# RobotLocomotion/pytorch-dense-correspondence

Hardware: NVIDIA H100
Metric: image-pairs/s (640x480, D=3) fwd+loss+bwd (higher is better)
Workload: dtype f32 (bf16x3 split on the wgmma tensor cores, fp32 accumulate)

## Files before the change

include/ddn_b200.h:

```cpp
#ifndef DDN_B200_H_
#define DDN_B200_H_

#include <stddef.h>
#include <stdint.h>

#ifdef __cplusplus
extern "C" {
#endif

#define DDN_ABI_VERSION 3

enum {
  DDN_OK = 0,
  DDN_EINVAL = -1,
  DDN_EWORKSPACE = -2,
  DDN_EUNSUPPORTED = -3
};

enum {
  DDN_PRECISION_FP32_SIMT = 0,
  DDN_PRECISION_BF16X3 = 1,
  DDN_PRECISION_BF16 = 2
};

// ... 151 lines not shown
                               float* five_host );

int ddn_conv2d_forward(const float* x_nhwc, const float* w_oihw, float* y_nhwc,
                       int N, int H, int W, int Cin, int Cout, int k, int stride, int pad, int dil,
                       int precision, void* workspace, size_t workspace_bytes, void* stream);
size_t ddn_conv2d_workspace_bytes(int N, int H, int W, int Cin, int Cout, int k, int stride, int pad, int dil, int precision);
int ddn_conv2d_backward(const float* x_nhwc, const float* w_oihw, const float* dy_nhwc,
                        float* dx_nhwc, float* dw_oihw,
                        int N, int H, int W, int Cin, int Cout, int k, int stride, int pad, int dil,
                        int precision, void* workspace, size_t workspace_bytes, void* stream);

int ddn_batchnorm_forward(const float* x, const float* gamma, const float* beta, const float* residual,
                          float* y, float* save_mean, float* save_invstd,
                          float* running_mean, float* running_var,
                          int64_t M, int C, int relu, int training, float momentum, float eps,
                          void* workspace, size_t workspace_bytes, void* stream);
int ddn_batchnorm_backward(const float* dy, const float* x, const float* y, const float* gamma,
                           const float* save_mean, const float* save_invstd,
                           float* dx, float* dgamma, float* dbeta, float* d_residual,
                           int64_t M, int C, int relu, void* workspace, size_t workspace_bytes, void* stream);
size_t ddn_batchnorm_workspace_bytes(int64_t M, int C);

size_t ddn_conv2d_fused_workspace_bytes(int N, int H, int W, int Cin, int Cout, int k, int stride, int pad, int dil, int precision);
int ddn_conv2d_bn_stats_forward(const float* x_nhwc, const float* w_oihw, float* raw_nhwc, float* mean, float* invstd,
                                float* running_mean, float* running_var,
                                int N, int H, int W, int Cin, int Cout, int k, int stride, int pad, int dil,
                                int bn_groups, float momentum, float eps, int precision,
                                void* workspace, size_t workspace_bytes, void* stream);
int ddn_conv2d_folded_forward(const float* x_nhwc, const float* w_oihw, const float* gamma, const float* beta,
                              const float* running_mean, const float* running_var, const float* addend_nhwc,
                              float* y_nhwc, void* y_hi_bf16, void* y_lo_bf16,
                              int N, int H, int W, int Cin, int Cout, int k, int stride, int pad, int dil, int relu, float eps,
                              int precision, void* workspace, size_t workspace_bytes, void* stream);
int ddn_conv2d_backward_data_bn_stats(const float* w_oihw, const float* dy_nhwc, const float* addend_nhwc,
                                      const float* raw_nhwc, const float* mean, const float* invstd, const float* gamma,
                                      const float* beta, const void* y_hi_bf16,
                                      float* dx_nhwc, float* dgamma, float* dbeta, float* sums,
                                      int N, int H, int W, int Cin, int Cout, int k, int stride, int pad, int dil,
                                      int bn_groups, int precision, void* workspace, size_t workspace_bytes, void* stream);

int ddn_stem_pool_forward(const float* raw, const float* mean, const float* invstd, const float* gamma, const float* beta,
                          float* y, void* y_hi_bf16, void* y_lo_bf16, void* argmax_u8, int N, int Hc, int Wc, int G, void* stream);
size_t ddn_stem_workspace_bytes(int N, int H, int W, int precision);
int ddn_stem_backward(const float* x_nchw, const float* raw, const float* mean, const float* invstd, const float* gamma,
                      const float* beta, const void* argmax_u8, const float* dy_pool, float* g_out, float* dx_bn,
                      void* dx_hi_bf16, void* dx_lo_bf16, float* dgamma, float* dbeta, float* dw_conv1,
// ... 188 lines not shown
```

pytorch-dense-correspondence_b200/_native.py:

```python
import ctypes
import os

import torch

_HERE = os.path.dirname(os.path.abspath(__file__))
LIB_PATH = os.path.join(_HERE, "libddn_b200.so")

PRECISION_FP32_SIMT, PRECISION_BF16X3, PRECISION_BF16 = 0, 1, 2
MODE_INFER, MODE_TRAIN, MODE_EVAL_SAVE = 0, 1, 2
ARCH_RESNET34_8S, ARCH_RESNET50_8S = 0, 1
GRAD_BUCKET_FN = ctypes.CFUNCTYPE(None, ctypes.c_void_p, ctypes.c_int, ctypes.c_int64, ctypes.c_int64)
TERM_MATCH, TERM_HINGE, TERM_HINGE_INV = 0, 1, 2
TERM_PIXEL_WEIGHT = 1
NET_UNIT_DESCRIPTORS = 1
LOWRES_UNIT = 1
MAX_TERMS = 8

c_f32p = ctypes.POINTER(ctypes.c_float)
vp, i32, i64, f32, sz = ctypes.c_void_p, ctypes.c_int, ctypes.c_int64, ctypes.c_float, ctypes.c_size_t


class TensorEntry(ctypes.Structure):
    _fields_ = [("name", ctypes.c_char * 64), ("ndim", ctypes.c_int32), ("shape", ctypes.c_int32 * 4),
                ("offset", ctypes.c_int64), ("numel", ctypes.c_int64)]
# ... 103 lines not shown
    "ddn_net_param_table": (i32, [i32, i32, ctypes.POINTER(TensorEntry), i32]),
    "ddn_net_buffer_table": (i32, [i32, ctypes.POINTER(TensorEntry), i32]),
    "ddn_net_param_count": (i64, [i32, i32]),
    "ddn_net_buffer_count": (i64, [i32]),
    "ddn_net_workspace_bytes": (sz, [i32] * 7),
    "ddn_net_weight_cache_bytes": (sz, [i32, i32]),
    "ddn_net_forward": (i32, [i32, vp, vp, vp, vp, vp, sz, i32, i32, i32, i32, i32, i32, f32, f32, i32, vp, vp]),
    "ddn_net_backward": (i32, [i32, vp, vp, vp, vp, vp, sz, i32, i32, i32, i32, i32, i32, f32, i32, GRAD_BUCKET_FN, vp, vp]),
    "ddn_net_grad_buckets": (i32, [i32, i32, ctypes.POINTER(i64), i32]),
    "ddn_net_workspace_bytes_v2": (sz, [i32] * 8),
    "ddn_net_forward_v2": (i32, [i32, vp, vp, vp, vp, vp, sz, i32, i32, i32, i32, i32, i32, f32, f32, i32, vp, i32, vp]),
    "ddn_net_backward_v2": (i32, [i32, vp, vp, vp, vp, vp, sz, i32, i32, i32, i32, i32, i32, f32, i32, i32, GRAD_BUCKET_FN, vp, vp]),
    "ddn_contrastive_terms_forward": (i32, [vp, vp, i64, i64, i64, i32, i64, i32, i32, ctypes.POINTER(LossTerm), i32, vp, vp, vp]),
    "ddn_contrastive_terms_backward": (i32, [vp, vp, i64, i64, i64, i32, i64, i32, i32, ctypes.POINTER(LossTerm), i32,
                                             vp, vp, vp, vp, vp]),
    "ddn_within_scene_compose": (i32, [vp, vp, i32, i32, ctypes.POINTER(WithinSceneCfg), vp, vp, vp]),
    "ddn_pair_type_compose": (i32, [vp, vp, i32, i32, ctypes.POINTER(PairTypeComposeCfg), vp, vp, vp, vp]),
    "ddn_within_scene_loss_host": (i32, [vp, vp, i32, i32, i32, i32, vp, vp, i64, vp, vp, i64, vp, vp, i64,
                                         f32, f32, f32, f32, i32, vp]),
    "ddn_conv2d_workspace_bytes": (sz, [i32] * 10),
    "ddn_conv2d_forward": (i32, [vp, vp, vp] + [i32] * 10 + [vp, sz, vp]),
    "ddn_conv2d_backward": (i32, [vp, vp, vp, vp, vp] + [i32] * 10 + [vp, sz, vp]),
    "ddn_conv2d_fused_workspace_bytes": (sz, [i32] * 10),
    "ddn_conv2d_bn_stats_forward": (i32, [vp] * 7 + [i32] * 10 + [f32, f32, i32, vp, sz, vp]),
    "ddn_conv2d_folded_forward": (i32, [vp] * 10 + [i32] * 10 + [f32, i32, vp, sz, vp]),
    "ddn_conv2d_backward_data_bn_stats": (i32, [vp] * 13 + [i32] * 11 + [vp, sz, vp]),
    "ddn_stem_pool_forward": (i32, [vp] * 9 + [i32] * 4 + [vp]),
    "ddn_stem_workspace_bytes": (sz, [i32] * 4),
    "ddn_stem_backward": (i32, [vp] * 15 + [i32] * 6 + [vp, sz, vp]),
    "ddn_batchnorm_workspace_bytes": (sz, [i64, i32]),
    "ddn_batchnorm_forward": (i32, [vp] * 9 + [i64, i32, i32, i32, f32, f32, vp, sz, vp]),
    "ddn_batchnorm_backward": (i32, [vp] * 10 + [i64, i32, i32, vp, sz, vp]),
    "ddn_upsample_bilinear_forward": (i32, [vp, vp, i32, i32, i32, i32, i32, vp]),
    "ddn_upsample_bilinear_backward": (i32, [vp, vp, i32, i32, i32, i32, i32, vp]),
    "ddn_upsample_bilinear_unit_forward": (i32, [vp, vp, i32, i32, i32, i32, i32, i32, vp]),
    "ddn_upsample_bilinear_unit_backward": (i32, [vp, vp, vp, vp, i32, i32, i32, i32, i32, i32, vp]),
    "ddn_fc_workspace_bytes": (sz, [i32, i32]),
    "ddn_fc_forward": (i32, [vp] * 7 + [i64, i32, i32, i32, vp]),
    "ddn_fc_backward": (i32, [vp] * 8 + [i64, i32, i32, i32, vp, sz, vp]),
    "ddn_scale_inplace": (i32, [vp, i64, f32, vp]),
    "ddn_sample_non_matches_scratch_bytes": (sz, [i32, i32]),
    "ddn_sample_non_matches": (i32, [vp, i32, i32, vp, vp, i64, vp, i64, vp, vp, vp, sz, vp]),
    "ddn_find_pixel_correspondences_scratch_bytes": (sz, [i64]),
    "ddn_find_pixel_correspondences": (i32, [vp, vp, i32, i32, vp, i64, vp, vp, vp, vp, vp, vp, vp, vp, vp, sz, vp]),
    "ddn_within_scene_batch_scratch_bytes": (sz, [ctypes.POINTER(WsBatchCfg)]),
    "ddn_within_scene_batch": (i32, [ctypes.POINTER(WsBatchCfg)] + [vp] * 9 + [ctypes.POINTER(WsBatchRand),
# ... 116 lines not shown
```

pytorch-dense-correspondence_b200/csrc/conv_tc.cu:

```cuda
#include <cuda.h>
#include <algorithm>
#include <cstring>
#include <functional>
#include <mutex>
#include <unordered_map>

#include "conv.cuh"
#include "conv_tc.cuh"

namespace ddn {

constexpr int TC_BLOCK_K = 64;
constexpr int TC_CONSUMERS = 256;
constexpr int TC_THREADS = TC_CONSUMERS + 32;
constexpr int TC_PRODUCER_WARP = TC_CONSUMERS / 32;
constexpr int TC_WIDE_THREADS = TC_CONSUMERS + 128;
constexpr int TC_A_BYTES = 128 * TC_BLOCK_K * 2;

__device__ __forceinline__ uint32_t smem_u32(const void* p) { return (uint32_t)__cvta_generic_to_shared(p); }

__device__ __forceinline__ void mbar_init(uint32_t bar, uint32_t count) {
  asm volatile("mbarrier.init.shared::cta.b64 [%0], %1;" ::"r"(bar), "r"(count));
}
__device__ __forceinline__ void mbar_expect_tx(uint32_t bar, uint32_t bytes) {
// ... 261 lines not shown

__device__ __forceinline__ void named_barrier(int id, int threads) { asm volatile("bar.sync %0, %1;" ::"r"(id), "r"(threads) : "memory"); }

__device__ __forceinline__ void conv_epilogue_finalize(const TcEpilogueParams& p, int C, int* s_last, int bar) {
  if (p.fin.a.acc) {
    if (bn_last_cta(p.fin.a.ticket, gridDim.x, threadIdx.x == 0, s_last, [bar] { named_barrier(bar, TC_CONSUMERS); }))
      for (int c = threadIdx.x; c < C; c += TC_CONSUMERS) bn_fwd_finalize_channel(p.fin, c);
  } else if (p.bst.fin.a.acc) {
    if (bn_last_cta(p.bst.fin.a.ticket, gridDim.x, threadIdx.x == 0, s_last, [bar] { named_barrier(bar, TC_CONSUMERS); }))
      for (int c = threadIdx.x; c < C; c += TC_CONSUMERS) bn_bwd_finalize_channel(p.bst.fin, c);
  }
}

struct TcConvParams {
  TcEpilogueParams epi;
  int N, H, W, Cin, Cout;
  int taps_w;
  int dil;
  int stride;
  int tiles_h, tiles_w;
  int n_sub;
  int n_co;
  int full_items, tail_split, total_items;
};

constexpr int TC_SUB_H = 4, TC_SUB_W = 16;
constexpr int TC_SUB_BYTES = 64 * 128;

struct TcItem { int sp, co0, width; };
__device__ __forceinline__ TcItem tc_item(const TcConvParams& p, int idx, int block_n) {
  int tile = idx, piece = 0, width = block_n;
  if (idx >= p.full_items) {
    const int j = idx - p.full_items;
    tile = p.full_items + j / p.tail_split;
    piece = j - (j / p.tail_split) * p.tail_split;
    width = block_n / p.tail_split;
  }
  TcItem it;
  it.sp = tile / p.n_co;
  it.co0 = (tile - it.sp * p.n_co) * block_n + piece * width;
  it.width = width;
  return it;
}
struct TcSub { int n, h0, w0; bool valid; };
__device__ __forceinline__ TcSub tc_sub(const TcConvParams& p, int st) {
  TcSub s;
  s.valid = st < p.n_sub;
  const int tw = st % p.tiles_w; const int t = st / p.tiles_w;
  const int th = t % p.tiles_h;
  s.n = s.valid ? t / p.tiles_h : p.N;
// ... 12 lines not shown
  constexpr int K_STEP = TRANS ? 16 * 128 : 32;
  for (int kb = 0; kb < num_kb; ++kb, ++g) {
    const int s = g % STAGES;
    mbar_wait(smem_u32(&full_bar[s]), (g / STAGES) & 1);
    wgmma_fence();
    const uint32_t stg = smem_u32(smem + (size_t)s * STAGE_BYTES);
    const uint64_t a_hi = gmma_desc(stg + wg * TC_SUB_BYTES, LBO, 1024), a_lo = gmma_desc(stg + A_BYTES + wg * TC_SUB_BYTES, LBO, 1024);
    const uint64_t b_hi = gmma_desc(stg + NSPLIT * A_BYTES, LBO, 1024), b_lo = gmma_desc(stg + 2 * A_BYTES + B_BYTES, LBO, 1024);
#pragma unroll
    for (int k = 0; k < TC_BLOCK_K / 16; ++k) {
      const uint64_t adv = (uint64_t)((k * K_STEP) >> 4);
      mma_k16_x<W, TRANS, NPROD>(acc, accx, a_hi + adv, a_lo + adv, b_hi + adv, b_lo + adv, (kb | k) != 0);
    }
    wgmma_commit();
    wgmma_wait<1>();
    if (kb > 0 && lane == 0) mbar_arrive(smem_u32(&empty_bar[(g - 1) % STAGES]));
  }
  wgmma_wait<0>();
  fence_acc(acc);
  if (NPROD == 3) { fence_acc(accx); add_cross(acc, accx); }
  if (lane == 0) mbar_arrive(smem_u32(&empty_bar[(g - 1) % STAGES]));
}

template <int BLOCK_N, int NPROD>
__global__ void __launch_bounds__(TC_WIDE_THREADS, 1)
conv_tc_kernel(const __grid_constant__ CUtensorMap tm_a_hi, const __grid_constant__ CUtensorMap tm_a_lo,
               const __grid_constant__ CUtensorMap tm_b_hi, const __grid_constant__ CUtensorMap tm_b_lo,
               const __grid_constant__ CUtensorMap tm_bt_hi, const __grid_constant__ CUtensorMap tm_bt_lo,
               const TcConvParams p) {
  constexpr int NSPLIT = NPROD == 3 ? 2 : 1;
  constexpr int A_BYTES = 128 * TC_BLOCK_K * 2;
  constexpr int B_BYTES = BLOCK_N * TC_BLOCK_K * 2;
  constexpr int STAGE_BYTES = NSPLIT * (A_BYTES + B_BYTES);
  constexpr int STAGES = (192 * 1024) / STAGE_BYTES >= 8 ? 8 : (192 * 1024) / STAGE_BYTES;
  static_assert(STAGES >= 2, "pipeline needs at least two stages");

  extern __shared__ __align__(1024) uint8_t smem_raw[];
  uint8_t* smem = reinterpret_cast<uint8_t*>((reinterpret_cast<uintptr_t>(smem_raw) + 1023) & ~uintptr_t(1023));
  __shared__ __align__(8) uint64_t full_bar[STAGES];
  __shared__ __align__(8) uint64_t empty_bar[STAGES];
  __shared__ int s_last;
  __shared__ __align__(16) float s_stage[TC_CONSUMERS / 32][EPI_WARP_FLOATS];
  __shared__ __align__(16) float s_part[2][2][4][BLOCK_N];

  pdl_trigger();
  const int warp = __shfl_sync(0xffffffffu, threadIdx.x >> 5, 0), lane = threadIdx.x & 31;
  const int cin_chunks = p.Cin / TC_BLOCK_K;
  const int num_kb = p.taps_w * p.taps_w * cin_chunks;
  const int half = p.taps_w >> 1;

  if (threadIdx.x == 0) {
    for (int s = 0; s < STAGES; ++s) { mbar_init(smem_u32(&full_bar[s]), 1); mbar_init(smem_u32(&empty_bar[s]), TC_CONSUMERS / 32); }
    fence_barrier_init();
    tma_prefetch_desc(&tm_a_hi); tma_prefetch_desc(&tm_b_hi); tma_prefetch_desc(&tm_bt_hi);
    if (NSPLIT == 2) { tma_prefetch_desc(&tm_a_lo); tma_prefetch_desc(&tm_b_lo); tma_prefetch_desc(&tm_bt_lo); }
  }
  __syncthreads();
  pdl_wait();

  if (warp >= TC_PRODUCER_WARP) {
    setmaxnreg_dec<40>();
    if (warp == TC_PRODUCER_WARP && lane == 0) {
      uint32_t g = 0;
      for (int idx = blockIdx.x; idx < p.total_items; idx += gridDim.x) {
        const TcItem it = tc_item(p, idx, BLOCK_N);
        const bool tail = it.width != BLOCK_N;
        const uint32_t stage_tx = (uint32_t)(NSPLIT * (A_BYTES + it.width * TC_BLOCK_K * 2));
        const CUtensorMap* mb_hi = tail ? &tm_bt_hi : &tm_b_hi;
        const CUtensorMap* mb_lo = tail ? &tm_bt_lo : &tm_b_lo;
        const TcSub s0 = tc_sub(p, it.sp * 2), s1 = tc_sub(p, it.sp * 2 + 1);
        for (int kb = 0; kb < num_kb; ++kb, ++g) {
          const int s = g % STAGES;
          mbar_wait(smem_u32(&empty_bar[s]), ((g / STAGES) & 1) ^ 1);
          const int tap = kb / cin_chunks, cc = kb - tap * cin_chunks;
          const int r = tap / p.taps_w, sx = tap - r * p.taps_w;
          const int dh = (r - half) * p.dil, dw = (sx - half) * p.dil;
          uint8_t* stg = smem + (size_t)s * STAGE_BYTES;
          const uint32_t bar = smem_u32(&full_bar[s]);
          mbar_expect_tx(bar, stage_tx);
          tma_load_4d(smem_u32(stg), &tm_a_hi, bar, cc * TC_BLOCK_K, s0.w0 * p.stride + dw, s0.h0 * p.stride + dh, s0.n);
          tma_load_4d(smem_u32(stg + TC_SUB_BYTES), &tm_a_hi, bar, cc * TC_BLOCK_K, s1.w0 * p.stride + dw, s1.h0 * p.stride + dh, s1.n);
          tma_load_2d(smem_u32(stg + NSPLIT * A_BYTES), mb_hi, bar, kb * TC_BLOCK_K, it.co0);
          if (NSPLIT == 2) {
            tma_load_4d(smem_u32(stg + A_BYTES), &tm_a_lo, bar, cc * TC_BLOCK_K, s0.w0 * p.stride + dw, s0.h0 * p.stride + dh, s0.n);
            tma_load_4d(smem_u32(stg + A_BYTES + TC_SUB_BYTES), &tm_a_lo, bar, cc * TC_BLOCK_K, s1.w0 * p.stride + dw, s1.h0 * p.stride + dh, s1.n);
            tma_load_2d(smem_u32(stg + 2 * A_BYTES + B_BYTES), mb_lo, bar, kb * TC_BLOCK_K, it.co0);
          }
        }
      }
    }
  } else {
    setmaxnreg_inc<232>();
    const int wg = warp >> 2, w = warp & 3, e = threadIdx.x & 127;
    const int ga = lane >> 3, gb = lane & 7;
    const bool stats = p.epi.fin.a.acc != nullptr;
    const bool bstats = p.epi.bst.fin.a.acc != nullptr;
    double* const sum_acc = bstats ? p.epi.bst.fin.a.acc : p.epi.fin.a.acc;
    float* const st = s_stage[warp];
    float acc[BLOCK_N / 2], accx[BLOCK_N / 2];
    uint32_t g = 0;
    for (int idx = blockIdx.x; idx < p.total_items; idx += gridDim.x) {
      const TcItem it = tc_item(p, idx, BLOCK_N);
      if (it.width == BLOCK_N)
        conv_tc_mainloop<BLOCK_N, BLOCK_N, NPROD, STAGES>(acc, accx, num_kb, g, full_bar, empty_bar, smem, wg, lane);
      else if (BLOCK_N > 64 && it.width == 64)
        conv_tc_mainloop<64, BLOCK_N, NPROD, STAGES>(acc_cols<64>(acc), acc_cols<64>(accx), num_kb, g, full_bar, empty_bar, smem, wg, lane);
      else
        conv_tc_mainloop<32, BLOCK_N, NPROD, STAGES>(acc_cols<32>(acc), acc_cols<32>(accx), num_kb, g, full_bar, empty_bar, smem, wg, lane);

      const TcSub sb = tc_sub(p, it.sp * 2 + wg);
      const int h = sb.h0 + w, w4 = sb.w0 + EPI_ROWS * ga;
      const int n_ok = (sb.valid && h < p.H) ? min(EPI_ROWS, p.W - w4) : 0;
      const size_t pix = ((size_t)(n_ok > 0 ? sb.n : 0) * p.H + (n_ok > 0 ? h : 0)) * p.W + (n_ok > 0 ? w4 : 0);
      const size_t cbase = pix * p.Cout + it.co0 + gb * 4;
      const int grp = sb.valid ? sb.n / p.epi.imgs_per_group : 0;
#pragma unroll
      for (int c = 0; c < BLOCK_N / 32; ++c) {
        if (c < (it.width >> 5)) {
          float4 v[EPI_ROWS];
          stage_chunk(acc, c, st, lane, v);
          float4 s1 = make_float4(0.f, 0.f, 0.f, 0.f), s2 = s1;
          conv_epilogue_rows(p.epi, v, cbase + c * 32, (size_t)p.Cout, n_ok, it.co0 + c * 32 + gb * 4, p.Cout, grp, s1, s2);
          if (stats || bstats) {
            colsum_lane_groups(s1, s2);
            if (ga == 0) {
              *reinterpret_cast<float4*>(&s_part[wg][0][w][c * 32 + gb * 4]) = s1;
              *reinterpret_cast<float4*>(&s_part[wg][1][w][c * 32 + gb * 4]) = s2;
            }
          }
        }
      }
      if (stats || bstats) {
        named_barrier(1 + wg, 128);
        if (sb.valid)
          for (int col = e; col < it.width; col += 128) {
#pragma unroll
            for (int k = 0; k < 2; ++k) {
              const float sum = s_part[wg][k][0][col] + s_part[wg][k][1][col] + s_part[wg][k][2][col] + s_part[wg][k][3][col];
              red_add_f64(sum_acc + (size_t)(grp * 2 + k) * p.Cout + it.co0 + col, (double)sum);
            }
          }
        named_barrier(1 + wg, 128);
      }
    }
    conv_epilogue_finalize(p.epi, p.Cout, &s_last, 3);
// ... 836 lines not shown
  DDN_CHECK_ARG(n % 4 == 0, "split: element count must be a multiple of 4");
  int64_t n4 = n / 4;
  int blocks = (int)std::min<int64_t>(ceil_div(n4, 256), (int64_t)num_sms() * 8);
  DDN_LAUNCH(split_bf16_kernel, blocks, 256, 0, st, x, hi, lo, n4, precision == DDN_PRECISION_BF16X3 ? 1 : 0);
  return 0;
}

int tc_upsample_zero_split(const float* dy, __nv_bfloat16* hi, __nv_bfloat16* lo, int N, int Ho, int Wo, int C, int precision,
                           cudaStream_t st) {
  int64_t total = (int64_t)N * Ho * Wo * (C / 4);
  int blocks = (int)std::min<int64_t>(ceil_div(total, 256), (int64_t)num_sms() * 8);
  DDN_LAUNCH(upsample_zero_split_kernel, blocks, 256, 0, st, dy, hi, lo, N, Ho, Wo, C, precision == DDN_PRECISION_BF16X3 ? 1 : 0);
  return 0;
}

int tc_stem_patches(const float* x_nchw, __nv_bfloat16* hi, __nv_bfloat16* lo, int N, int H, int W, int precision, cudaStream_t st) {
  const int H1 = (H - 1) / 2 + 1, W1 = (W - 1) / 2 + 1;
  DDN_CHECK_ARG(N <= 65535 && H1 <= 65535, "stem: batch / height too large for the launch grid");
  dim3 grid((unsigned)ceil_div(W1, STEM_TW), (unsigned)H1, (unsigned)N);
  DDN_LAUNCH(stem_patch_split_kernel, grid, 256, 0, st, x_nchw, hi, lo, N, H, W, H1, W1, precision == DDN_PRECISION_BF16X3 ? 1 : 0);
  return 0;
}

template <int BLOCK_N, int NPROD>
static int launch_conv_tc(const CUtensorMap& a_hi, const CUtensorMap& a_lo, const CUtensorMap& b_hi, const CUtensorMap& b_lo,
                          const CUtensorMap& bt_hi, const CUtensorMap& bt_lo, const TcConvParams& p, int workers, cudaStream_t st) {
  constexpr int NSPLIT = NPROD == 3 ? 2 : 1;
  constexpr int STAGE_BYTES = NSPLIT * (128 * TC_BLOCK_K * 2 + BLOCK_N * TC_BLOCK_K * 2);
  constexpr int STAGES = (192 * 1024) / STAGE_BYTES >= 8 ? 8 : (192 * 1024) / STAGE_BYTES;
  const size_t smem = (size_t)STAGES * STAGE_BYTES + 1024;
  static bool configured = false;
  if (!configured) {
    DDN_CUDA(cudaFuncSetAttribute(conv_tc_kernel<BLOCK_N, NPROD>, cudaFuncAttributeMaxDynamicSharedMemorySize, (int)smem));
    configured = true;
  }
  DDN_LAUNCH((conv_tc_kernel<BLOCK_N, NPROD>), workers, TC_WIDE_THREADS, smem, st, a_hi, a_lo, b_hi, b_lo, bt_hi, bt_lo, p);
  return 0;
}

template <int NPROD>
static int launch_conv64_halo(const CUtensorMap& a_hi, const CUtensorMap& a_lo, const CUtensorMap& b_hi, const CUtensorMap& b_lo,
                              const TcHaloParams& p, cudaStream_t st) {
  constexpr int NSPLIT = NPROD == 3 ? 2 : 1;
  const size_t smem = (size_t)NSPLIT * HALO_B_PLANE + (size_t)halo_slots(NPROD) * HALO_SLOT + 1024;
  static bool configured = false;
  if (!configured) {
    DDN_CUDA(cudaFuncSetAttribute(conv64_halo_kernel<NPROD>, cudaFuncAttributeMaxDynamicSharedMemorySize, (int)smem));
    configured = true;
  }
  const int grid = std::min(p.n_tiles, tc_worker_sms());
  DDN_LAUNCH((conv64_halo_kernel<NPROD>), grid, TC_THREADS, smem, st, a_hi, a_lo, b_hi, b_lo, p);
  return 0;
}

static int tc_epilogue_request(TcEpilogueParams* e, float* out, const float* addend, const BnFwdFinal* stats, const TcBwdStats* bst,
                               const TcFoldedEpilogue* ep, int N, int gout, int dgrad, int want_lo) {
  memset(e, 0, sizeof(*e));
  e->out = out; e->addend = addend; e->imgs_per_group = N;
  if (stats) {
// ... 54 lines not shown
    DDN_TRY(make_weight_map(&mb_lo, want_lo ? b_lo : b_hi, 64, 9 * 64, 64));
    ProfScope ps(dgrad ? PROF_CONV_DGRAD_TC : PROF_CONV_FWD_TC, fl, st);
    return want_lo ? launch_conv64_halo<3>(ma_hi, ma_lo, mb_hi, mb_lo, hp, st) : launch_conv64_halo<1>(ma_hi, ma_lo, mb_hi, mb_lo, hp, st);
  }
  const int block_n = gout % 128 == 0 ? 128 : 64;
  TcConvParams p;
  memset(&p, 0, sizeof(p));
  p.epi = epi; p.N = N; p.H = Ho; p.W = Wo; p.Cin = gin; p.Cout = gout; p.taps_w = k; p.dil = dil;
  p.stride = stride;
  p.tiles_h = (int)ceil_div(Ho, TC_SUB_H); p.tiles_w = (int)ceil_div(Wo, TC_SUB_W);
  p.n_sub = N * p.tiles_h * p.tiles_w;
  p.n_co = gout / block_n;
  const int tiles = (int)ceil_div(p.n_sub, 2) * p.n_co;
  const int workers_max = tc_worker_sms();
  const int rem = tiles % workers_max;
  int split = 1;
  if (rem)
    while (split * 2 <= 8 && block_n / (split * 2) >= 32 && rem * split * 2 <= workers_max) split *= 2;
  p.full_items = tiles - rem; p.tail_split = split; p.total_items = p.full_items + rem * split;
  if (split == 1) { p.full_items = tiles; p.total_items = tiles; }
  const int workers = std::min(p.total_items, workers_max);
  const int b_rows = block_n;
  const int bt_rows = b_rows / split;
  CUtensorMap ma_hi, ma_lo, mb_hi, mb_lo, mt_hi, mt_lo;
  DDN_TRY(make_act_map(&ma_hi, in.hi, N, H, W, gin, stride));
  DDN_TRY(make_act_map(&ma_lo, want_lo ? in.lo : in.hi, N, H, W, gin, stride));
  DDN_TRY(make_weight_map(&mb_hi, b_hi, gout, k * k * gin, b_rows));
  DDN_TRY(make_weight_map(&mb_lo, want_lo ? b_lo : b_hi, gout, k * k * gin, b_rows));
  DDN_TRY(make_weight_map(&mt_hi, b_hi, gout, k * k * gin, bt_rows));
  DDN_TRY(make_weight_map(&mt_lo, want_lo ? b_lo : b_hi, gout, k * k * gin, bt_rows));
  ProfScope ps(dgrad ? PROF_CONV_DGRAD_TC : PROF_CONV_FWD_TC, fl, st);
#define CONV_TC(BN)                                                                                                           \
  (want_lo ? launch_conv_tc<BN, 3>(ma_hi, ma_lo, mb_hi, mb_lo, mt_hi, mt_lo, p, workers, st)                                   \
           : launch_conv_tc<BN, 1>(ma_hi, ma_lo, mb_hi, mb_lo, mt_hi, mt_lo, p, workers, st))
  if (block_n == 128) return CONV_TC(128);
  return CONV_TC(64);
#undef CONV_TC
}

int tc_dgrad_strided(const float* dy_f32, TcPlanes up, const float* w_oihw, const TcPlanes* w_packed, float* dx, const float* addend,
                     int N, int H, int W, int Cin, int Cout, int k, int precision, void* wws, size_t wws_bytes, cudaStream_t st,
                     const TcBwdStats* bst) {
  DDN_TRY(tc_upsample_zero_split(dy_f32, const_cast<__nv_bfloat16*>(up.hi), const_cast<__nv_bfloat16*>(up.lo), N, H / 2, W / 2, Cout,
                                 precision, st));
  return tc_conv_planes(up, w_oihw, w_packed, dx, addend, nullptr, N, H, W, Cin, Cout, k, 1, 1, 1, precision, wws, wws_bytes, st, nullptr, bst);
}

int tc_stem_pack_weights(const float* w_conv1, __nv_bfloat16* hi, __nv_bfloat16* lo, int precision, cudaStream_t st) {
  DDN_LAUNCH(stem_pack_weights_kernel, (64 * 192 + 255) / 256, 256, 0, st, w_conv1, hi, lo, precision == DDN_PRECISION_BF16X3 ? 1 : 0);
  return 0;
}
int tc_stem_forward(TcPlanes patches, const float* w_conv1, const TcPlanes* w_packed, float* raw, const BnFwdFinal* stats, int N, int H1,
                    int W1, int precision, void* wws, size_t wws_bytes, cudaStream_t st) {
  TcPlanes wpk;
  if (w_packed) wpk = *w_packed;
  else {
    char* base = reinterpret_cast<char*>(align_up(reinterpret_cast<uintptr_t>(wws), 1024));
    DDN_CHECK_ARG((size_t)(base - (char*)wws) + 2 * 64 * 192 * 2 + 1024 <= wws_bytes, "weight staging too small");
    __nv_bfloat16* ph = (__nv_bfloat16*)base; __nv_bfloat16* pl = (__nv_bfloat16*)(base + align_up((size_t)64 * 192 * 2, 1024));
// ... 71 lines not shown
```

pytorch-dense-correspondence_b200/csrc/conv_tc.cuh:

```cuda
#pragma once
#include "common.cuh"
#include "bn_stats.cuh"

namespace ddn {

struct TcPlanes { const __nv_bfloat16* hi; const __nv_bfloat16* lo; };

struct TcFoldedEpilogue { const float* scale; const float* shift; int relu; __nv_bfloat16* out_hi; __nv_bfloat16* out_lo; };

struct TcBwdStats {
  const float* raw; const __nv_bfloat16* y_hi;
  const float* mean; const float* invstd;
  const float* gamma; const float* beta;
  int relu;
  BnBwdFinal fin;
};

bool tc_conv_supported(int Cin, int Cout, int k, int stride, int pad, int dil, int H, int W);
size_t tc_weight_ws_bytes();
size_t tc_max_weight_elems();
size_t tc_workspace_bytes(size_t max_act_elems);
int tc_split(const float* x, __nv_bfloat16* hi, __nv_bfloat16* lo, int64_t n, int precision, cudaStream_t st);

int tc_conv_planes(TcPlanes in, const float* w_oihw, const TcPlanes* w_packed, float* out, const float* addend, const BnFwdFinal* stats,
                   int N, int H, int W, int Cin, int Cout, int k, int stride, int dil, int dgrad, int precision,
                   void* wws, size_t wws_bytes, cudaStream_t st, const TcFoldedEpilogue* ep = nullptr, const TcBwdStats* bst = nullptr);
int tc_dgrad_strided(const float* dy_f32, TcPlanes up, const float* w_oihw, const TcPlanes* w_packed, float* dx, const float* addend,
                     int N, int H, int W, int Cin, int Cout, int k, int precision, void* wws, size_t wws_bytes, cudaStream_t st,
                     const TcBwdStats* bst = nullptr);
int tc_wgrad_planes(TcPlanes x, TcPlanes dy, float* dw, int N, int H, int W, int Cin, int Cout, int k, int stride, int dil,
                    int precision, double* dwp, cudaStream_t st);
struct TcUnpackEntry { int64_t src_off, dst_off; int Cout, Cin, taps, kind; };
constexpr int TC_UNPACK_MAX = 40;
struct TcUnpackTable { TcUnpackEntry e[TC_UNPACK_MAX]; int n; };
int tc_unpack_wgrads(const TcUnpackEntry* entries, int n, const double* dwp_base, float* grads_base, cudaStream_t st);
struct TcPackEntry { int64_t w_off, dst_off; int Cout, Cin, k, dgrad, kind; };
constexpr int TC_PACK_MAX = 80;
struct TcPackTable { TcPackEntry e[TC_PACK_MAX]; int n; };
int tc_pack_all(const float* params, int64_t n_params, char* cache, const TcPackEntry* entries, int n, unsigned long long* fp_new,
                unsigned long long* fp_old, int force, int precision, cudaStream_t st);
int tc_stem_patches(const float* x_nchw, __nv_bfloat16* hi, __nv_bfloat16* lo, int N, int H, int W, int precision, cudaStream_t st);
int tc_stem_pack_weights(const float* w_conv1, __nv_bfloat16* hi, __nv_bfloat16* lo, int precision, cudaStream_t st);
// ... 13 lines not shown
```

pytorch-dense-correspondence_b200/csrc/engine.cu:

```cuda
#include <algorithm>
#include <cstring>
#include <deque>
#include <mutex>
#include <string>
#include <vector>

#include "conv.cuh"
#include "conv_tc.cuh"

namespace ddn {

std::atomic<long long> g_launches{0};
static thread_local char g_err[512] = "";

void set_error(const char* fmt, ...) {
  va_list ap;
  va_start(ap, fmt);
  vsnprintf(g_err, sizeof(g_err), fmt, ap);
  va_end(ap);
}

static std::atomic<int> g_reserved_sms{-1};
static std::atomic<int> g_window_reserved{0};
static int overlap_window_sms() {
// ... 963 lines not shown
  BnBwdArgs a;
  memset(&a, 0, sizeof(a));
  a.dy = dy; a.x = x; a.mean = save_mean; a.invstd = save_invstd; a.gamma = gamma; a.y = y;
  a.dx = dx; a.g_out = d_residual; a.dgamma = dgamma; a.dbeta = dbeta;
  a.acc = bn_accum_at(workspace, C); a.sums = reinterpret_cast<float*>((char*)workspace + bn_accum_bytes(C));
  a.M = M; a.C = C; a.relu = relu; a.training = 1; a.G = 1;
  return launch_bn_backward(a, st);
}

static bool is_stem_shape(int Cin, int Cout, int k, int stride, int pad, int dil) {
  return Cin == 3 && Cout == 64 && k == 7 && stride == 2 && pad == 3 && dil == 1;
}
static size_t fused_head_bytes(int C) { return bn_accum_bytes(C) + align_up(sizeof(float) * 2 * (size_t)C, 256); }

extern "C" size_t ddn_conv2d_fused_workspace_bytes(int N, int H, int W, int Cin, int Cout, int k, int stride, int pad, int dil,
                                                   int precision) {
  if (N < 1 || H < 1 || W < 1 || Cin < 1 || Cout < 1 || precision == DDN_PRECISION_FP32_SIMT) return 0;
  const int C = Cin > Cout ? Cin : Cout;
  size_t act = (size_t)N * H * W * C;
  if (is_stem_shape(Cin, Cout, k, stride, pad, dil)) act = (size_t)N * conv_out(H, 7, 2, 3, 1) * conv_out(W, 7, 2, 3, 1) * 192;
  return fused_head_bytes(C) + tc_workspace_bytes(act) + 1024;
}

static int check_fused(int N, int H, int W, int Cin, int Cout, int k, int stride, int pad, int dil, int G, int precision,
                       size_t ws_bytes, bool allow_stem) {
  DDN_CHECK_ARG(precision >= DDN_PRECISION_FP32_SIMT && precision <= DDN_PRECISION_BF16, "unknown precision %d", precision);
  if (precision == DDN_PRECISION_FP32_SIMT) {
    set_error("the fused conv epilogues exist on the tensor-core path only (precision %d)", precision);
    return DDN_EUNSUPPORTED;
  }
  DDN_CHECK_ARG(N >= 1 && H >= 8 && W >= 8, "bad sizes N=%d H=%d W=%d", N, H, W);
  DDN_CHECK_ARG(G >= 1 && G <= BN_MAX_GROUPS && N % G == 0, "bn_groups must be 1 or %d and divide N (got %d for N=%d)", BN_MAX_GROUPS, G, N);
  const bool stem = is_stem_shape(Cin, Cout, k, stride, pad, dil);
  if (stem) {
    if (!allow_stem) { set_error("the stem patch GEMM has no fused variant here"); return DDN_EUNSUPPORTED; }
  } else if (!tc_conv_supported(Cin, Cout, k, stride, pad, dil, H, W)) {
    set_error("shape not supported by the tensor-core path (Cin=%d Cout=%d k=%d stride=%d pad=%d dil=%d H=%d W=%d)", Cin, Cout, k, stride,
              pad, dil, H, W);
    return DDN_EUNSUPPORTED;
  }
  DDN_CHECK_ARG(ws_bytes >= ddn_conv2d_fused_workspace_bytes(N, H, W, Cin, Cout, k, stride, pad, dil, precision), "workspace too small");
  return 0;
}

extern "C" int ddn_conv2d_bn_stats_forward(const float* x, const float* w, float* raw, float* mean, float* invstd, float* running_mean,
                                           float* running_var, int N, int H, int W, int Cin, int Cout, int k, int stride, int pad,
// ... 158 lines not shown
```

Baseline: 139.6.

## Load one haloed activation row box per kernel row for 3x3 dgrad convs

For stride-1 3x3 data-gradient convolutions, the producer now loads one wider activation box per kernel row (with dilation halo) and reuses it for all three horizontal taps by shifting the wgmma descriptor. Activation and weight tiles get separate mbarrier rings, with weights still streamed per tap. This cuts activation TMA traffic about threefold for these layers. In exchange, the shared-memory split and epilogue indexing change (column-major sub-tile rows), which adds complexity and leaves fewer weight stages.

```diff
diff --git a/include/ddn_b200.h b/include/ddn_b200.h
--- a/include/ddn_b200.h
+++ b/include/ddn_b200.h
@@ -197,6 +197,7 @@
 size_t ddn_batchnorm_workspace_bytes(int64_t M, int C);
 
 size_t ddn_conv2d_fused_workspace_bytes(int N, int H, int W, int Cin, int Cout, int k, int stride, int pad, int dil, int precision);
+int ddn_conv_tc_load_bytes(int k, int stride, int dil, int dgrad, int width, int precision, int64_t* out);
 int ddn_conv2d_bn_stats_forward(const float* x_nhwc, const float* w_oihw, float* raw_nhwc, float* mean, float* invstd,
                                 float* running_mean, float* running_var,
                                 int N, int H, int W, int Cin, int Cout, int k, int stride, int pad, int dil,
diff --git a/pytorch-dense-correspondence_b200/_native.py b/pytorch-dense-correspondence_b200/_native.py
--- a/pytorch-dense-correspondence_b200/_native.py
+++ b/pytorch-dense-correspondence_b200/_native.py
@@ -149,6 +149,7 @@
     "ddn_conv2d_forward": (i32, [vp, vp, vp] + [i32] * 10 + [vp, sz, vp]),
     "ddn_conv2d_backward": (i32, [vp, vp, vp, vp, vp] + [i32] * 10 + [vp, sz, vp]),
     "ddn_conv2d_fused_workspace_bytes": (sz, [i32] * 10),
+    "ddn_conv_tc_load_bytes": (i32, [i32] * 6 + [vp]),
     "ddn_conv2d_bn_stats_forward": (i32, [vp] * 7 + [i32] * 10 + [f32, f32, i32, vp, sz, vp]),
     "ddn_conv2d_folded_forward": (i32, [vp] * 10 + [i32] * 10 + [f32, i32, vp, sz, vp]),
     "ddn_conv2d_backward_data_bn_stats": (i32, [vp] * 13 + [i32] * 11 + [vp, sz, vp]),
diff --git a/pytorch-dense-correspondence_b200/csrc/conv_tc.cu b/pytorch-dense-correspondence_b200/csrc/conv_tc.cu
--- a/pytorch-dense-correspondence_b200/csrc/conv_tc.cu
+++ b/pytorch-dense-correspondence_b200/csrc/conv_tc.cu
@@ -307,10 +307,26 @@
   int n_sub;
   int n_co;
   int full_items, tail_split, total_items;
+  uint32_t a_tx, b_tx, bt_tx;
 };
 
 constexpr int TC_SUB_H = 4, TC_SUB_W = 16;
 constexpr int TC_SUB_BYTES = 64 * 128;
+
+constexpr int TC_ROW_MAX_DIL = 4;
+constexpr int TC_ROW_BOX_MAX = TC_SUB_H * (TC_SUB_W + 2 * TC_ROW_MAX_DIL) * 128;
+
+template <int BLOCK_N, int NPROD, bool ROWS>
+struct TcRing {
+  static constexpr int NSPLIT = NPROD == 3 ? 2 : 1;
+  static constexpr int B_BYTES = BLOCK_N * TC_BLOCK_K * 2;
+  static constexpr int A_SLOT = ROWS ? NSPLIT * 2 * TC_ROW_BOX_MAX : 0;
+  static constexpr int A_SLOTS = ROWS ? (96 * 1024) / A_SLOT : 0;
+  static constexpr int B_SLOT = NSPLIT * ((ROWS ? 0 : TC_A_BYTES) + B_BYTES);
+  static constexpr int B_SLOTS = (192 * 1024 - A_SLOTS * A_SLOT) / B_SLOT >= 8 ? 8 : (192 * 1024 - A_SLOTS * A_SLOT) / B_SLOT;
+  static constexpr int SMEM = A_SLOTS * A_SLOT + B_SLOTS * B_SLOT + 1024;
+  static_assert(B_SLOTS >= 2 && (!ROWS || A_SLOTS >= 2), "pipeline needs at least two stages");
+};
 
 struct TcItem { int sp, co0, width; };
 __device__ __forceinline__ TcItem tc_item(const TcConvParams& p, int idx, int block_n) {
@@ -369,23 +385,67 @@
   if (lane == 0) mbar_arrive(smem_u32(&empty_bar[(g - 1) % STAGES]));
 }
 
-template <int BLOCK_N, int NPROD>
+template <int W, class R>
+__device__ __forceinline__ void conv_tc_mainloop_rows(float (&acc)[W / 2], float (&accx)[W / 2], int num_rows, int dil, uint32_t& ga,
+                                                      uint32_t& g, const uint64_t* a_full, const uint64_t* a_empty, const uint64_t* b_full,
+                                                      const uint64_t* b_empty, const uint8_t* smem, int wg, int lane) {
+  constexpr int NPROD = R::NSPLIT == 2 ? 3 : 1;
+  const uint32_t tap_shift = (uint32_t)(dil * TC_SUB_H * 128) >> 4;
+  for (int j = 0; j < num_rows; ++j, ++ga) {
+    const int sa = ga % R::A_SLOTS;
+    mbar_wait(smem_u32(&a_full[sa]), (ga / R::A_SLOTS) & 1);
+    const uint32_t abase = smem_u32(smem + (size_t)sa * R::A_SLOT) + wg * TC_ROW_BOX_MAX;
+    const uint64_t a_hi0 = gmma_desc_k(abase), a_lo0 = gmma_desc_k(abase + 2 * TC_ROW_BOX_MAX);
+#pragma unroll
+    for (int s = 0; s < 3; ++s, ++g) {
+      const int sb = g % R::B_SLOTS;
+      mbar_wait(smem_u32(&b_full[sb]), (g / R::B_SLOTS) & 1);
+      wgmma_fence();
+      const uint32_t bbase = smem_u32(smem + (size_t)R::A_SLOTS * R::A_SLOT + (size_t)sb * R::B_SLOT);
+      const uint64_t b_hi = gmma_desc_k(bbase), b_lo = gmma_desc_k(bbase + R::B_BYTES);
+      const uint64_t a_hi = a_hi0 + s * tap_shift, a_lo = a_lo0 + s * tap_shift;
+#pragma unroll
+      for (int k = 0; k < TC_BLOCK_K / 16; ++k) {
+        const uint64_t adv = (uint64_t)((k * 32) >> 4);
+        mma_k16_x<W, 0, NPROD>(acc, accx, a_hi + adv, a_lo + adv, b_hi + adv, b_lo + adv, (j | s | k) != 0);
+      }
+      wgmma_commit();
+      wgmma_wait<1>();
+      if (lane == 0 && (j | s) != 0) {
+        mbar_arrive(smem_u32(&b_empty[(g - 1) % R::B_SLOTS]));
+        if (s == 0) mbar_arrive(smem_u32(&a_empty[(ga - 1) % R::A_SLOTS]));
+      }
+    }
+  }
+  wgmma_wait<0>();
+  fence_acc(acc);
+  if (NPROD == 3) { fence_acc(accx); add_cross(acc, accx); }
+  if (lane == 0) {
+    mbar_arrive(smem_u32(&b_empty[(g - 1) % R::B_SLOTS]));
+    mbar_arrive(smem_u32(&a_empty[(ga - 1) % R::A_SLOTS]));
+  }
+}
+
+template <int BLOCK_N, int NPROD, bool ROWS>
 __global__ void __launch_bounds__(TC_WIDE_THREADS, 1)
 conv_tc_kernel(const __grid_constant__ CUtensorMap tm_a_hi, const __grid_constant__ CUtensorMap tm_a_lo,
                const __grid_constant__ CUtensorMap tm_b_hi, const __grid_constant__ CUtensorMap tm_b_lo,
                const __grid_constant__ CUtensorMap tm_bt_hi, const __grid_constant__ CUtensorMap tm_bt_lo,
                const TcConvParams p) {
-  constexpr int NSPLIT = NPROD == 3 ? 2 : 1;
-  constexpr int A_BYTES = 128 * TC_BLOCK_K * 2;
-  constexpr int B_BYTES = BLOCK_N * TC_BLOCK_K * 2;
-  constexpr int STAGE_BYTES = NSPLIT * (A_BYTES + B_BYTES);
-  constexpr int STAGES = (192 * 1024) / STAGE_BYTES >= 8 ? 8 : (192 * 1024) / STAGE_BYTES;
-  static_assert(STAGES >= 2, "pipeline needs at least two stages");
+  using R = TcRing<BLOCK_N, NPROD, ROWS>;
+  constexpr int NSPLIT = R::NSPLIT;
+  constexpr int A_BYTES = TC_A_BYTES;
+  constexpr int B_BYTES = R::B_BYTES;
+  constexpr int STAGE_BYTES = R::B_SLOT;
+  constexpr int STAGES = R::B_SLOTS;
+  constexpr int A_SLOTS = ROWS ? R::A_SLOTS : 1;
 
   extern __shared__ __align__(1024) uint8_t smem_raw[];
   uint8_t* smem = reinterpret_cast<uint8_t*>((reinterpret_cast<uintptr_t>(smem_raw) + 1023) & ~uintptr_t(1023));
   __shared__ __align__(8) uint64_t full_bar[STAGES];
   __shared__ __align__(8) uint64_t empty_bar[STAGES];
+  __shared__ __align__(8) uint64_t a_full_bar[A_SLOTS];
+  __shared__ __align__(8) uint64_t a_empty_bar[A_SLOTS];
   __shared__ int s_last;
   __shared__ __align__(16) float s_stage[TC_CONSUMERS / 32][EPI_WARP_FLOATS];
   __shared__ __align__(16) float s_part[2][2][4][BLOCK_N];
@@ -394,10 +454,13 @@
   const int warp = __shfl_sync(0xffffffffu, threadIdx.x >> 5, 0), lane = threadIdx.x & 31;
   const int cin_chunks = p.Cin / TC_BLOCK_K;
   const int num_kb = p.taps_w * p.taps_w * cin_chunks;
+  const int num_rows = 3 * cin_chunks;
   const int half = p.taps_w >> 1;
 
   if (threadIdx.x == 0) {
     for (int s = 0; s < STAGES; ++s) { mbar_init(smem_u32(&full_bar[s]), 1); mbar_init(smem_u32(&empty_bar[s]), TC_CONSUMERS / 32); }
+    if (ROWS)
+      for (int s = 0; s < A_SLOTS; ++s) { mbar_init(smem_u32(&a_full_bar[s]), 1); mbar_init(smem_u32(&a_empty_bar[s]), TC_CONSUMERS / 32); }
     fence_barrier_init();
     tma_prefetch_desc(&tm_a_hi); tma_prefetch_desc(&tm_b_hi); tma_prefetch_desc(&tm_bt_hi);
     if (NSPLIT == 2) { tma_prefetch_desc(&tm_a_lo); tma_prefetch_desc(&tm_b_lo); tma_prefetch_desc(&tm_bt_lo); }
@@ -408,14 +471,44 @@
   if (warp >= TC_PRODUCER_WARP) {
     setmaxnreg_dec<40>();
     if (warp == TC_PRODUCER_WARP && lane == 0) {
-      uint32_t g = 0;
+      uint32_t g = 0, ga = 0;
       for (int idx = blockIdx.x; idx < p.total_items; idx += gridDim.x) {
         const TcItem it = tc_item(p, idx, BLOCK_N);
         const bool tail = it.width != BLOCK_N;
-        const uint32_t stage_tx = (uint32_t)(NSPLIT * (A_BYTES + it.width * TC_BLOCK_K * 2));
+        const uint32_t b_tx = tail ? p.bt_tx : p.b_tx;
         const CUtensorMap* mb_hi = tail ? &tm_bt_hi : &tm_b_hi;
         const CUtensorMap* mb_lo = tail ? &tm_bt_lo : &tm_b_lo;
         const TcSub s0 = tc_sub(p, it.sp * 2), s1 = tc_sub(p, it.sp * 2 + 1);
+        if constexpr (ROWS) {
+          uint8_t* const smem_b = smem + (size_t)R::A_SLOTS * R::A_SLOT;
+          for (int j = 0; j < num_rows; ++j, ++ga) {
+            const int r = j / cin_chunks, cc = j - r * cin_chunks;
+            const int sa = ga % A_SLOTS;
+            mbar_wait(smem_u32(&a_empty_bar[sa]), ((ga / A_SLOTS) & 1) ^ 1);
+            uint8_t* const as = smem + (size_t)sa * R::A_SLOT;
+            const uint32_t abar = smem_u32(&a_full_bar[sa]);
+            const int dh = (r - 1) * p.dil;
+            mbar_expect_tx(abar, p.a_tx);
+            tma_load_4d(smem_u32(as), &tm_a_hi, abar, cc * TC_BLOCK_K, s0.h0 + dh, s0.w0 - p.dil, s0.n);
+            tma_load_4d(smem_u32(as + TC_ROW_BOX_MAX), &tm_a_hi, abar, cc * TC_BLOCK_K, s1.h0 + dh, s1.w0 - p.dil, s1.n);
+            if (NSPLIT == 2) {
+              tma_load_4d(smem_u32(as + 2 * TC_ROW_BOX_MAX), &tm_a_lo, abar, cc * TC_BLOCK_K, s0.h0 + dh, s0.w0 - p.dil, s0.n);
+              tma_load_4d(smem_u32(as + 3 * TC_ROW_BOX_MAX), &tm_a_lo, abar, cc * TC_BLOCK_K, s1.h0 + dh, s1.w0 - p.dil, s1.n);
+            }
+            for (int sx = 0; sx < 3; ++sx, ++g) {
+              const int s = g % STAGES;
+              mbar_wait(smem_u32(&empty_bar[s]), ((g / STAGES) & 1) ^ 1);
+              uint8_t* const bs = smem_b + (size_t)s * STAGE_BYTES;
+              const uint32_t bar = smem_u32(&full_bar[s]);
+              const int kcol = (r * 3 + sx) * p.Cin + cc * TC_BLOCK_K;
+              mbar_expect_tx(bar, b_tx);
+              tma_load_2d(smem_u32(bs), mb_hi, bar, kcol, it.co0);
+              if (NSPLIT == 2) tma_load_2d(smem_u32(bs + B_BYTES), mb_lo, bar, kcol, it.co0);
+            }
+          }
+          continue;
+        }
+        const uint32_t stage_tx = p.a_tx + b_tx;
         for (int kb = 0; kb < num_kb; ++kb, ++g) {
           const int s = g % STAGES;
           mbar_wait(smem_u32(&empty_bar[s]), ((g / STAGES) & 1) ^ 1);
@@ -445,20 +538,40 @@
     double* const sum_acc = bstats ? p.epi.bst.fin.a.acc : p.epi.fin.a.acc;
     float* const st = s_stage[warp];
     float acc[BLOCK_N / 2], accx[BLOCK_N / 2];
-    uint32_t g = 0;
+    uint32_t g = 0, gra = 0;
     for (int idx = blockIdx.x; idx < p.total_items; idx += gridDim.x) {
       const TcItem it = tc_item(p, idx, BLOCK_N);
-      if (it.width == BLOCK_N)
-        conv_tc_mainloop<BLOCK_N, BLOCK_N, NPROD, STAGES>(acc, accx, num_kb, g, full_bar, empty_bar, smem, wg, lane);
-      else if (BLOCK_N > 64 && it.width == 64)
-        conv_tc_mainloop<64, BLOCK_N, NPROD, STAGES>(acc_cols<64>(acc), acc_cols<64>(accx), num_kb, g, full_bar, empty_bar, smem, wg, lane);
-      else
-        conv_tc_mainloop<32, BLOCK_N, NPROD, STAGES>(acc_cols<32>(acc), acc_cols<32>(accx), num_kb, g, full_bar, empty_bar, smem, wg, lane);
+      if constexpr (ROWS) {
+        if (it.width == BLOCK_N)
+          conv_tc_mainloop_rows<BLOCK_N, R>(acc, accx, num_rows, p.dil, gra, g, a_full_bar, a_empty_bar, full_bar, empty_bar, smem, wg, lane);
+        else if (BLOCK_N > 64 && it.width == 64)
+          conv_tc_mainloop_rows<64, R>(acc_cols<64>(acc), acc_cols<64>(accx), num_rows, p.dil, gra, g, a_full_bar, a_empty_bar, full_bar,
+                                       empty_bar, smem, wg, lane);
+        else
+          conv_tc_mainloop_rows<32, R>(acc_cols<32>(acc), acc_cols<32>(accx), num_rows, p.dil, gra, g, a_full_bar, a_empty_bar, full_bar,
+                                       empty_bar, smem, wg, lane);
+      } else {
+        if (it.width == BLOCK_N)
+          conv_tc_mainloop<BLOCK_N, BLOCK_N, NPROD, STAGES>(acc, accx, num_kb, g, full_bar, empty_bar, smem, wg, lane);
+        else if (BLOCK_N > 64 && it.width == 64)
+          conv_tc_mainloop<64, BLOCK_N, NPROD, STAGES>(acc_cols<64>(acc), acc_cols<64>(accx), num_kb, g, full_bar, empty_bar, smem, wg, lane);
+        else
+          conv_tc_mainloop<32, BLOCK_N, NPROD, STAGES>(acc_cols<32>(acc), acc_cols<32>(accx), num_kb, g, full_bar, empty_bar, smem, wg, lane);
+      }
 
       const TcSub sb = tc_sub(p, it.sp * 2 + wg);
-      const int h = sb.h0 + w, w4 = sb.w0 + EPI_ROWS * ga;
-      const int n_ok = (sb.valid && h < p.H) ? min(EPI_ROWS, p.W - w4) : 0;
-      const size_t pix = ((size_t)(n_ok > 0 ? sb.n : 0) * p.H + (n_ok > 0 ? h : 0)) * p.W + (n_ok > 0 ? w4 : 0);
+      int n_ok, h, wc;
+      size_t rs;
+      if constexpr (ROWS) {
+        h = sb.h0; wc = sb.w0 + 4 * w + ga;
+        n_ok = (sb.valid && wc < p.W) ? min(EPI_ROWS, p.H - h) : 0;
+        rs = (size_t)p.W * p.Cout;
+      } else {
+        h = sb.h0 + w; wc = sb.w0 + EPI_ROWS * ga;
+        n_ok = (sb.valid && h < p.H) ? min(EPI_ROWS, p.W - wc) : 0;
+        rs = (size_t)p.Cout;
+      }
+      const size_t pix = ((size_t)(n_ok > 0 ? sb.n : 0) * p.H + (n_ok > 0 ? h : 0)) * p.W + (n_ok > 0 ? wc : 0);
       const size_t cbase = pix * p.Cout + it.co0 + gb * 4;
       const int grp = sb.valid ? sb.n / p.epi.imgs_per_group : 0;
 #pragma unroll
@@ -467,7 +580,7 @@
           float4 v[EPI_ROWS];
           stage_chunk(acc, c, st, lane, v);
           float4 s1 = make_float4(0.f, 0.f, 0.f, 0.f), s2 = s1;
-          conv_epilogue_rows(p.epi, v, cbase + c * 32, (size_t)p.Cout, n_ok, it.co0 + c * 32 + gb * 4, p.Cout, grp, s1, s2);
+          conv_epilogue_rows(p.epi, v, cbase + c * 32, rs, n_ok, it.co0 + c * 32 + gb * 4, p.Cout, grp, s1, s2);
           if (stats || bstats) {
             colsum_lane_groups(s1, s2);
             if (ga == 0) {
@@ -1350,19 +1463,29 @@
   return 0;
 }
 
-template <int BLOCK_N, int NPROD>
+bool tc_row_boxes(int k, int stride, int dil, int dgrad) { return dgrad && k == 3 && stride == 1 && dil >= 1 && dil <= TC_ROW_MAX_DIL; }
+
+TcLoadBytes tc_load_bytes(int k, int stride, int dil, int dgrad, int width, int precision) {
+  const int nsplit = precision == DDN_PRECISION_BF16X3 ? 2 : 1;
+  TcLoadBytes b;
+  const bool rows = tc_row_boxes(k, stride, dil, dgrad);
+  const int box_pixels = rows ? TC_SUB_H * (TC_SUB_W + 2 * dil) : TC_SUB_H * TC_SUB_W;
+  b.a = nsplit * 2 * box_pixels * TC_BLOCK_K * 2;
+  b.a_kblocks = rows ? 3 : 1;
+  b.b = nsplit * width * TC_BLOCK_K * 2;
+  return b;
+}
+
+template <int BLOCK_N, int NPROD, bool ROWS>
 static int launch_conv_tc(const CUtensorMap& a_hi, const CUtensorMap& a_lo, const CUtensorMap& b_hi, const CUtensorMap& b_lo,
                           const CUtensorMap& bt_hi, const CUtensorMap& bt_lo, const TcConvParams& p, int workers, cudaStream_t st) {
-  constexpr int NSPLIT = NPROD == 3 ? 2 : 1;
-  constexpr int STAGE_BYTES = NSPLIT * (128 * TC_BLOCK_K * 2 + BLOCK_N * TC_BLOCK_K * 2);
-  constexpr int STAGES = (192 * 1024) / STAGE_BYTES >= 8 ? 8 : (192 * 1024) / STAGE_BYTES;
-  const size_t smem = (size_t)STAGES * STAGE_BYTES + 1024;
+  const size_t smem = TcRing<BLOCK_N, NPROD, ROWS>::SMEM;
   static bool configured = false;
   if (!configured) {
-    DDN_CUDA(cudaFuncSetAttribute(conv_tc_kernel<BLOCK_N, NPROD>, cudaFuncAttributeMaxDynamicSharedMemorySize, (int)smem));
+    DDN_CUDA(cudaFuncSetAttribute(conv_tc_kernel<BLOCK_N, NPROD, ROWS>, cudaFuncAttributeMaxDynamicSharedMemorySize, (int)smem));
     configured = true;
   }
-  DDN_LAUNCH((conv_tc_kernel<BLOCK_N, NPROD>), workers, TC_WIDE_THREADS, smem, st, a_hi, a_lo, b_hi, b_lo, bt_hi, bt_lo, p);
+  DDN_LAUNCH((conv_tc_kernel<BLOCK_N, NPROD, ROWS>), workers, TC_WIDE_THREADS, smem, st, a_hi, a_lo, b_hi, b_lo, bt_hi, bt_lo, p);
   return 0;
 }
 
@@ -1463,19 +1586,27 @@
   const int workers = std::min(p.total_items, workers_max);
   const int b_rows = block_n;
   const int bt_rows = b_rows / split;
+  const bool rows = tc_row_boxes(k, stride, dil, dgrad);
+  const TcLoadBytes lb = tc_load_bytes(k, stride, dil, dgrad, b_rows, precision), lbt = tc_load_bytes(k, stride, dil, dgrad, bt_rows, precision);
+  p.a_tx = (uint32_t)lb.a; p.b_tx = (uint32_t)lb.b; p.bt_tx = (uint32_t)lbt.b;
   CUtensorMap ma_hi, ma_lo, mb_hi, mb_lo, mt_hi, mt_lo;
-  DDN_TRY(make_act_map(&ma_hi, in.hi, N, H, W, gin, stride));
-  DDN_TRY(make_act_map(&ma_lo, want_lo ? in.lo : in.hi, N, H, W, gin, stride));
+  if (rows) {
+    DDN_TRY(make_act_map_hw(&ma_hi, in.hi, N, H, W, gin, TC_SUB_H, TC_SUB_W + 2 * dil));
+    DDN_TRY(make_act_map_hw(&ma_lo, want_lo ? in.lo : in.hi, N, H, W, gin, TC_SUB_H, TC_SUB_W + 2 * dil));
+  } else {
+    DDN_TRY(make_act_map(&ma_hi, in.hi, N, H, W, gin, stride));
+    DDN_TRY(make_act_map(&ma_lo, want_lo ? in.lo : in.hi, N, H, W, gin, stride));
+  }
   DDN_TRY(make_weight_map(&mb_hi, b_hi, gout, k * k * gin, b_rows));
   DDN_TRY(make_weight_map(&mb_lo, want_lo ? b_lo : b_hi, gout, k * k * gin, b_rows));
   DDN_TRY(make_weight_map(&mt_hi, b_hi, gout, k * k * gin, bt_rows));
   DDN_TRY(make_weight_map(&mt_lo, want_lo ? b_lo : b_hi, gout, k * k * gin, bt_rows));
   ProfScope ps(dgrad ? PROF_CONV_DGRAD_TC : PROF_CONV_FWD_TC, fl, st);
-#define CONV_TC(BN)                                                                                                           \
-  (want_lo ? launch_conv_tc<BN, 3>(ma_hi, ma_lo, mb_hi, mb_lo, mt_hi, mt_lo, p, workers, st)                                   \
-           : launch_conv_tc<BN, 1>(ma_hi, ma_lo, mb_hi, mb_lo, mt_hi, mt_lo, p, workers, st))
-  if (block_n == 128) return CONV_TC(128);
-  return CONV_TC(64);
+#define CONV_TC(BN, ROWS)                                                                                                     \
+  (want_lo ? launch_conv_tc<BN, 3, ROWS>(ma_hi, ma_lo, mb_hi, mb_lo, mt_hi, mt_lo, p, workers, st)                             \
+           : launch_conv_tc<BN, 1, ROWS>(ma_hi, ma_lo, mb_hi, mb_lo, mt_hi, mt_lo, p, workers, st))
+  if (rows) return block_n == 128 ? CONV_TC(128, true) : CONV_TC(64, true);
+  return block_n == 128 ? CONV_TC(128, false) : CONV_TC(64, false);
 #undef CONV_TC
 }
 
diff --git a/pytorch-dense-correspondence_b200/csrc/conv_tc.cuh b/pytorch-dense-correspondence_b200/csrc/conv_tc.cuh
--- a/pytorch-dense-correspondence_b200/csrc/conv_tc.cuh
+++ b/pytorch-dense-correspondence_b200/csrc/conv_tc.cuh
@@ -18,6 +18,9 @@
 
 bool tc_conv_supported(int Cin, int Cout, int k, int stride, int pad, int dil, int H, int W);
 size_t tc_weight_ws_bytes();
+bool tc_row_boxes(int k, int stride, int dil, int dgrad);
+struct TcLoadBytes { int a, a_kblocks, b; };
+TcLoadBytes tc_load_bytes(int k, int stride, int dil, int dgrad, int width, int precision);
 size_t tc_max_weight_elems();
 size_t tc_workspace_bytes(size_t max_act_elems);
 int tc_split(const float* x, __nv_bfloat16* hi, __nv_bfloat16* lo, int64_t n, int precision, cudaStream_t st);
diff --git a/pytorch-dense-correspondence_b200/csrc/engine.cu b/pytorch-dense-correspondence_b200/csrc/engine.cu
--- a/pytorch-dense-correspondence_b200/csrc/engine.cu
+++ b/pytorch-dense-correspondence_b200/csrc/engine.cu
@@ -1009,6 +1009,17 @@
   return fused_head_bytes(C) + tc_workspace_bytes(act) + 1024;
 }
 
+extern "C" int ddn_conv_tc_load_bytes(int k, int stride, int dil, int dgrad, int width, int precision, int64_t* out) {
+  DDN_CHECK_ARG(out != nullptr, "null output");
+  DDN_CHECK_ARG((k == 1 || k == 3) && (stride == 1 || stride == 2) && dil >= 1 && (dgrad == 0 || dgrad == 1) &&
+                (width == 32 || width == 64 || width == 128) && !(dgrad && stride != 1),
+                "bad conv k=%d stride=%d dil=%d dgrad=%d width=%d", k, stride, dil, dgrad, width);
+  DDN_CHECK_ARG(precision == DDN_PRECISION_BF16X3 || precision == DDN_PRECISION_BF16, "tensor-core precision only, got %d", precision);
+  const TcLoadBytes b = tc_load_bytes(k, stride, dil, dgrad, width, precision);
+  out[0] = b.a; out[1] = b.a_kblocks; out[2] = b.b;
+  return 0;
+}
+
 static int check_fused(int N, int H, int W, int Cin, int Cout, int k, int stride, int pad, int dil, int G, int precision,
                        size_t ws_bytes, bool allow_stem) {
   DDN_CHECK_ARG(precision >= DDN_PRECISION_FP32_SIMT && precision <= DDN_PRECISION_BF16, "unknown precision %d", precision);
```

New measurement: 141.5 (median of 6 runs). 1.4% higher.
